# jonasrothfuss/meta_learning_pacoh

Measured on AMD Instinct MI355X. Metric: task-GP LML+grad evals/sec (n_ctx=64, d=4, 20 particles), higher is better.
Workload: dtype f32; 1 GPU; PACOH-SVGD step as meta_fit runs it (hipGraph replay), cfg#3: 1024 tasks per GPU x 20 particles, n_ctx=64, d=4, NN(32,32) mean + NN(32,32) kernel (D=2534), task sharding + 1 all-reduce/step; parallelism=task-shard x1, finite=True, tasks_total=1024, particles=20, n_ctx=64, d=4

## Files before the change

meta_learning_pacoh_amd/csrc/gp_fwd_reg.hip:

```cpp
#include "gp_reg_body.h"
#include "mlp_act.h"
#include "step_tail.h"
#include "switches.h"

namespace pacoh {

struct FwdGpArgs {
    const float* x;
    const float* theta; long theta_stride;
    long off_mean, off_kern;
    float* stash_mean; float* stash_kern;
    int d_in, h0, h1;
    int nblk;
    unsigned n_prob;
    SvgdDistTail<float> sv;
};

namespace gpreg {

struct FwdCtx : KernelCtx {
    static constexpr bool LDS_INPUTS = true;
    __device__ __forceinline__ int lane() const { int l = threadIdx.x; asm volatile("" : "+v"(l)); return l; }
};

__device__ __forceinline__ void dist_tail_wave(const SvgdDistTail<float>& t, int lin, int nlin) {
    const int lane = threadIdx.x;
    if (lin == 0 && lane == 0 && t.counter) *t.counter += 1;
    for (int pair = lin; pair < t.P * t.P; pair += nlin) {
        const int i = pair / t.P, j = pair - i * t.P;
        if (j > i) continue;
        const float* xi = t.X + (long)i * t.D;
        if (t.snap && i == j) {
            for (int d = lane; d < t.D; d += 64) t.snap[(long)i * t.D + d] = xi[d];
            if (lane == 0) t.d2[i * t.P + i] = 0.0f;
            continue;
        }
        const float* xj = t.X + (long)j * t.D;
        float acc[4] = {0.0f, 0.0f, 0.0f, 0.0f};
        for (int d0 = lane; d0 < t.D; d0 += 256) {
#pragma unroll
            for (int w = 0; w < 4; ++w) {
                const int d = d0 + 64 * w;
                if (d < t.D) { const float df = xi[d] - xj[d]; acc[w] = fmaf(df, df, acc[w]); }
            }
        }
#pragma unroll
        for (int w = 0; w < 4; ++w) acc[w] = subwave_sum<float>(acc[w], 64);
        if (lane == 0) { const float tot = (acc[0] + acc[1]) + (acc[2] + acc[3]); t.d2[i * t.P + j] = tot; t.d2[j * t.P + i] = tot; }
    }
}

template <int NH, bool W32, bool MEAN>
__device__ __forceinline__ void fwd_net(const float* __restrict__ th, const FwdGpArgs& fa, int d_out, const float (&bx)[4], float* stash,
                                        long blk0, int lane, float* zf, float* rv) {
    const int r = lane & 15, g = lane >> 4;
    const int h0 = W32 ? 32 : fa.h0, d_in = fa.d_in;
    float aw1[2];
    f32x4 b1[2];
#pragma unroll
    for (int fb = 0; fb < 2; ++fb) {
        const int o = fb * 16 + r;
        aw1[fb] = ((W32 || o < h0) && g < d_in) ? TSC * th[h0 + o * d_in + g] : 0.0f;
#pragma unroll
        for (int s = 0; s < 4; ++s) { const int q = fb * 16 + 4 * g + s; b1[fb][s] = (W32 || q < h0) ? TSC * th[q] : 0.0f; }
    }
    int src = h0 * (d_in + 1), prev = h0;
    f32x4 aw2[2][2], b2[2];
    if constexpr (NH == 2) {
        const int hl = W32 ? 32 : fa.h1;
#pragma unroll
        for (int ob = 0; ob < 2; ++ob) {
            const int o = ob * 16 + r;
#pragma unroll
            for (int kb = 0; kb < 2; ++kb)
#pragma unroll
                for (int j = 0; j < 4; ++j) {
                    const int k = kb * 16 + 4 * g + j;
                    aw2[ob][kb][j] = (W32 || (o < hl && k < prev)) ? TSC * th[src + hl + o * prev + k] : 0.0f;
                }
#pragma unroll
            for (int s = 0; s < 4; ++s) { const int q = ob * 16 + 4 * g + s; b2[ob][s] = (W32 || q < hl) ? TSC * th[src + q] : 0.0f; }
        }
        src += hl * (prev + 1);
        prev = hl;
    }
    constexpr int NO = MEAN ? 1 : 2;
    float w3[NO][2][4], b3[NO];
#pragma unroll
    for (int o = 0; o < NO; ++o) {
        b3[o] = o < d_out ? th[src + o] : 0.0f;
#pragma unroll
        for (int fb = 0; fb < 2; ++fb)
#pragma unroll
            for (int s = 0; s < 4; ++s) {
                const int k = fb * 16 + 4 * g + s;
                w3[o][fb][s] = (o < d_out && (W32 || k < prev)) ? th[src + d_out + o * prev + k] : 0.0f;
            }
    }
#pragma unroll
    for (int pb = 0; pb < 4; ++pb) {
        asm volatile("" ::: "memory"); __builtin_amdgcn_sched_barrier(0);
        f32x4 HA[2], HB[2];
#pragma unroll
        for (int fb = 0; fb < 2; ++fb) {
            f32x4 acc = mfma_(aw1[fb], bx[pb], b1[fb]);
#pragma unroll
            for (int s = 0; s < 4; ++s) acc[s] = tanh_pre(acc[s]);
            HA[fb] = acc;
        }
        if constexpr (NH == 2) {
#pragma unroll
            for (int ob = 0; ob < 2; ++ob) {
                f32x4 acc = b2[ob];
#pragma unroll
                for (int kb = 0; kb < 2; ++kb) {
                    acc = mfma_(aw2[ob][kb][0], HA[kb][0], acc); acc = mfma_(aw2[ob][kb][1], HA[kb][1], acc);
                    acc = mfma_(aw2[ob][kb][2], HA[kb][2], acc); acc = mfma_(aw2[ob][kb][3], HA[kb][3], acc);
                }
#pragma unroll
                for (int s = 0; s < 4; ++s) acc[s] = tanh_pre(acc[s]);
                HB[ob] = acc;
            }
            if (stash) {
#pragma unroll
                for (int fb = 0; fb < 2; ++fb)
                    __builtin_nontemporal_store(HB[fb], reinterpret_cast<f32x4*>(stash + ((((blk0 + pb) * 2 + fb) << 8) + (lane << 2))));
            }
        }
        const f32x4 (&HL)[2] = NH == 2 ? HB : HA;
        float v[NO];
#pragma unroll
        for (int o = 0; o < NO; ++o) v[o] = 0.0f;
#pragma unroll
        for (int fb = 0; fb < 2; ++fb)
#pragma unroll
            for (int s = 0; s < 4; ++s)
#pragma unroll
                for (int o = 0; o < NO; ++o) v[o] = fmaf(w3[o][fb][s], HL[fb][s], v[o]);
#pragma unroll
        for (int o = 0; o < NO; ++o) { v[o] += __shfl_xor(v[o], 16, 64); v[o] += __shfl_xor(v[o], 32, 64); }
        if (g == 0) {
            if constexpr (MEAN) rv[pb * 16 + r] = v[0] + b3[0];
            else {
                zf[(pb * 16 + r) * 2] = v[0] + b3[0];
                if (d_out > 1) zf[(pb * 16 + r) * 2 + 1] = v[1] + b3[1];
            }
        }
    }
}

}

template <int NH, bool W32>
__global__ void __launch_bounds__(64, 4) gp_fwd_reg_kernel(GpMfmaArgs a, FwdGpArgs fa) {
    if (blockIdx.x >= fa.n_prob) {
        gpreg::dist_tail_wave(fa.sv, (int)(blockIdx.x - fa.n_prob), (int)(gridDim.x - fa.n_prob));
        return;
    }
    if (const int32_t* n_act = gpreg::KernelCtx{}.late(a.n_act, (unsigned)__builtin_offsetof(GpMfmaArgs, n_act))) {
        if (blockIdx.x >= (unsigned)*n_act * (unsigned)a.P) return;
    }
    constexpr int NB = 4, FP = 2, NP = 16 * NB, NU = NB * (NB + 1) / 2;
    __shared__ __attribute__((aligned(16))) float zf[NP * FP];
    __shared__ __attribute__((aligned(16))) float rv[NP];
    __shared__ __attribute__((aligned(16))) float av[NP];
    __shared__ __attribute__((aligned(16))) float fsc[gpreg::GPR_SCR];
    float* tsc = fsc;
    __shared__ __attribute__((aligned(16))) float dzc[NP * FP];
    __shared__ __attribute__((aligned(16))) float Wl[(NU - NB) * 256];
    {
        const int lane = threadIdx.x, r = lane & 15, g = lane >> 4;
        const unsigned t = blockIdx.x / (unsigned)a.P, p = blockIdx.x - t * (unsigned)a.P;
        const float* xt = fa.x + (long)t * NP * fa.d_in;
        float bx[4];
#pragma unroll
        for (int pb = 0; pb < 4; ++pb) bx[pb] = g < fa.d_in ? xt[(pb * 16 + r) * fa.d_in + g] : 0.0f;
        const float* th = fa.theta + (long)p * fa.theta_stride;
        const long blk0 = (long)p * fa.nblk + 4 * t;
        gpreg::fwd_net<NH, W32, true>(th + fa.off_mean, fa, 1, bx, fa.stash_mean, blk0, lane, zf, rv);
        asm volatile("" ::: "memory"); __builtin_amdgcn_sched_barrier(0);
        gpreg::fwd_net<NH, W32, false>(th + fa.off_kern, fa, a.f, bx, fa.stash_kern, blk0, lane, zf, rv);
        asm volatile("" ::: "memory"); __builtin_amdgcn_wave_barrier();
    }
    gpreg::gp_reg_body<NB, FP, true, false>(a, gpreg::FwdCtx{}, zf, rv, av, fsc, tsc, dzc, Wl);
}

static bool fwd_gp_applicable(int B, int P, int n, int x_div, int d_in, const int32_t* hidden, int n_hidden, int f_arg, int has_os,
                              int mean_mode, int dtype) {
    if (dtype != PACOH_F32 || kernel_of(f_arg) != PACOH_KERNEL_RBF || has_os || mean_mode != PACOH_MEAN_VECTOR) return false;
    const int f = features_of(f_arg);
    if (f < 1 || f > 2 || n != 64 || P <= 0 || B <= 0 || B % P != 0 || x_div != P || d_in < 1 || d_in > 4) return false;
    if (n_hidden < 1 || n_hidden > 2 || !hidden || g_sw.mlp_path != 0) return false;
    for (int l = 0; l < n_hidden; ++l) if (hidden[l] < 1 || hidden[l] > 32) return false;
    return (long)B * n <= 0x3fffffffL;
}

}

using namespace pacoh;

extern "C" int pacoh_fwd_gp_applicable(int B, int P, int n, int x_div, int d_in, const int32_t* hidden, int n_hidden, int f,
                                       int has_outputscale, int mean_mode, int dtype) {
    return fwd_gp_applicable(B, P, n, x_div, d_in, hidden, n_hidden, f, has_outputscale, mean_mode, dtype) ? 1 : 0;
}

extern "C" int pacoh_fwd_gp_lml_fwdbwd(const pacoh_active_tasks* act, const void* x, int x_div, const void* theta, long theta_stride, int P,
                                       int d_in, const int32_t* hidden, int n_hidden, long off_mean, long off_kernel, void* stash,
                                       const void* svgd_X, void* svgd_workspace, int svgd_P, int svgd_D, int64_t* counter,
                                       const void* y, int y_div, const void* lengthscale, const void* outputscale, const void* noise,
                                       const int32_t* n_valid, const void* g_lml, void* lml, void* d_z, void* d_mean,
                                       void* d_lengthscale, void* d_outputscale, void* d_noise, int32_t* info,
                                       int B, int n, int f, int dtype, void* stream) {
    if (check_dtype(dtype)) return PACOH_EDTYPE;
    if (!x || !theta || !y || !lengthscale || !noise || !lml || !d_lengthscale || !d_noise || y_div <= 0 || off_mean < 0 || off_kernel < 0)
        return PACOH_EINVAL;
    if (act && (!act->n_act || !act->task_w)) return PACOH_EINVAL;
    if (svgd_X && (!svgd_workspace || svgd_P <= 0 || svgd_D <= 0)) return PACOH_EINVAL;
    if (svgd_X && svgd_P > PACOH_SVGD_MAX_PARTICLES) return PACOH_ELIMIT;
    if (!fwd_gp_applicable(B, P, n, x_div, d_in, hidden, n_hidden, f, outputscale != nullptr || d_outputscale != nullptr,
                           PACOH_MEAN_VECTOR, dtype))
        return PACOH_ELIMIT;
    GpMfmaArgs a = {nullptr, 1, nullptr, PACOH_MEAN_VECTOR, (const float*)y, y_div, (const float*)lengthscale, nullptr, (const float*)noise,
                    n_valid, (const float*)g_lml, (float*)lml, info, (float*)d_z, (float*)d_mean, (float*)d_lengthscale, nullptr,
                    (float*)d_noise, B, P, n, features_of(f)};
    if (act) { a.n_act = act->n_act; a.task_w = (const float*)act->task_w; }
    FwdGpArgs fa = {};
    fa.x = (const float*)x; fa.theta = (const float*)theta; fa.theta_stride = theta_stride;
    fa.off_mean = off_mean; fa.off_kern = off_kernel;
    fa.d_in = d_in; fa.h0 = hidden[0]; fa.h1 = n_hidden > 1 ? hidden[1] : 0;
    fa.nblk = 4 * (B / P);
    if (stash && n_hidden > 1) {
        fa.stash_mean = (float*)stash;
        fa.stash_kern = (float*)stash + (size_t)P * fa.nblk * 2 * 256;
    }
    fa.n_prob = (unsigned)B;
    unsigned tail_wgs = 0;
    if (svgd_X) {
        float* d2 = (float*)svgd_workspace;
        fa.sv = SvgdDistTail<float>{(const float*)svgd_X, d2, d2 + svgd_P * svgd_P, svgd_P, svgd_D, (long*)counter};
        tail_wgs = (unsigned)(svgd_P * svgd_P);
    }
    const bool w32 = hidden[0] == 32 && (n_hidden == 1 || hidden[1] == 32);
    const dim3 grid((unsigned)B + tail_wgs);
    hipStream_t s = (hipStream_t)stream;
    if (n_hidden == 2) {
        if (w32) hipLaunchKernelGGL((gp_fwd_reg_kernel<2, true>), grid, dim3(64), 0, s, a, fa);
        else hipLaunchKernelGGL((gp_fwd_reg_kernel<2, false>), grid, dim3(64), 0, s, a, fa);
    } else {
        if (w32) hipLaunchKernelGGL((gp_fwd_reg_kernel<1, true>), grid, dim3(64), 0, s, a, fa);
        else hipLaunchKernelGGL((gp_fwd_reg_kernel<1, false>), grid, dim3(64), 0, s, a, fa);
    }
    return launch_status();
}
```

meta_learning_pacoh_amd/csrc/mlp_fused.hip:

```cpp
#include "common.h"
#include "hyper_tail.h"
#include "step_tail.h"
#include "mlp_fused_split.h"
#include "mlp_act.h"
#include <stdlib.h>

namespace pacoh {

using f32x4 = __attribute__((ext_vector_type(4))) float;

constexpr int FMAXNH = 4;
constexpr int LWH = 36;
constexpr int HBLK = 32 * LWH + 32;
constexpr int F_OFF_W1 = 0;
constexpr int F_OFF_B1 = 128;
constexpr int F_OFF_H = 160;
__host__ __device__ constexpr int f_off_out(int nh) { return F_OFF_H + (nh - 1) * HBLK; }
__host__ __device__ constexpr int f_welems(int nh) { return f_off_out(nh) + 68; }
__host__ __device__ constexpr int f_dnet_max(int nh) { return 32 * 5 + (nh - 1) * 32 * 33 + 2 * 33; }
__host__ __device__ constexpr bool bwd_wg_slab(int nh) { return nh <= 2; }
constexpr int TSTRIDE = 4;
constexpr int TSTAGE = 6;
constexpr int TLD = 17;
__host__ __device__ constexpr int tskew(int k) { return 12 * (k & 1) + 32 * (k >> 1); }
constexpr int TRS = 320;

struct FusedNet {
    long theta_off;
    float* out;
    const float* g_out;
    float* slab;
    float* stash;
    int d_out, D_net;
};

struct FusedArgs {
    const float* x; int x_div;
    const float* theta; long theta_stride;
    FusedNet net[2];
    int P, n, R;
    int d_in, nh;
    int h[FMAXNH];
    int tiles_per_wg;
    int n_stash;
    int nblk;
    int tail_z;
    SvgdDistTail<float> sv;
    const float* bw_d2; float* bw_out; int bw_P;
    long* adv_counter;
    const int32_t* n_act;
    int tiles;
};

__device__ __forceinline__ void fused_live_rows(const FusedArgs& a, int tp, int& R, int& tpw) {
    R = a.R; tpw = a.tiles_per_wg;
    if (!a.n_act) return;
    const int live = *a.n_act * a.n;
    if (live < R) R = live;
    tpw = fused_split_tiles((R + tp - 1) / tp, a.tiles, (int)gridDim.x, tpw);
}

__device__ __forceinline__ long stash_off(const FusedArgs& a, int p, int blk, int slot, int fb, int lane) {
    return (((((long)p * a.nblk + blk) * a.n_stash + slot) * 2 + fb) << 8) + (lane << 2);
}

__device__ __forceinline__ f32x4 fmfma(float a, float b, f32x4 c) {
    return __builtin_amdgcn_mfma_f32_16x16x4f32(a, b, c, 0, 0, 0);
}


template <int NH>
__device__ void fused_load_weights(float* wl, const float* __restrict__ th, const FusedArgs& a, int d_out) {
    for (int q = threadIdx.x; q < f_welems(NH); q += blockDim.x) wl[q] = 0.0f;
    __syncthreads();
    int src = 0;
    const int h0 = a.h[0], d_in = a.d_in;
    for (int q = threadIdx.x; q < h0; q += blockDim.x) wl[F_OFF_B1 + q] = TSC * th[q];
    for (int q = threadIdx.x; q < h0 * d_in; q += blockDim.x) { const int o = q / d_in, k = q - o * d_in; wl[F_OFF_W1 + o * 4 + k] = TSC * th[h0 + q]; }
    src += h0 * (d_in + 1);
    int prev = h0;
#pragma unroll
    for (int l = 1; l < NH; ++l) {
        const int hl = a.h[l];
        float* dst = wl + F_OFF_H + (l - 1) * HBLK;
        for (int q = threadIdx.x; q < hl; q += blockDim.x) dst[32 * LWH + q] = TSC * th[src + q];
        for (int q = threadIdx.x; q < hl * prev; q += blockDim.x) { const int o = q / prev, k = q - o * prev; dst[o * LWH + k] = TSC * th[src + hl + q]; }
        src += hl * (prev + 1);
        prev = hl;
    }
    float* dst = wl + f_off_out(NH);
    for (int q = threadIdx.x; q < d_out; q += blockDim.x) dst[64 + q] = th[src + q];
    for (int q = threadIdx.x; q < d_out * prev; q += blockDim.x) { const int o = q / prev, k = q - o * prev; dst[o * 32 + k] = th[src + d_out + q]; }
    __syncthreads();
}

template <int PB, bool BWD>
__device__ __forceinline__ long stage_tile(const FusedArgs& a, const FusedNet& nt, int p, int row0, float* st, int lane, int R) {
    long orow = -1;
    if (lane < 16 * PB) {
        const int row = row0 + lane;
        const bool valid = row < R;
        const int rr = valid ? row : R - 1;
        const int t = (int)((unsigned)rr / (unsigned)a.n), i = rr - t * a.n;
        const int bi = t * a.P + p;
        const int xb = a.x_div == 1 ? bi : (int)((unsigned)bi / (unsigned)a.x_div);
        const float* xq = a.x + ((long)xb * a.n + i) * (long)a.d_in;
        float4 xv;
        xv.x = xq[0];
        xv.y = a.d_in > 1 ? xq[1] : 0.0f;
        xv.z = a.d_in > 2 ? xq[2] : 0.0f;
        xv.w = a.d_in > 3 ? xq[3] : 0.0f;
        *reinterpret_cast<float4*>(st + lane * TSTRIDE) = xv;
        const long o = (long)bi * a.n + i;
        if (BWD) {
            const float* gq = nt.g_out + o * nt.d_out;
            st[16 * PB * TSTRIDE + lane] = valid ? gq[0] : 0.0f;
            st[16 * PB * (TSTRIDE + 1) + lane] = (valid && nt.d_out > 1) ? gq[1] : 0.0f;
        }
        orow = valid ? o : -1;
    }
    asm volatile("" ::: "memory");
    return orow;
}

template <int PB>
__device__ __forceinline__ void f_layer1(const float* wl, const float* st, int r, int g, f32x4 (&H)[2][PB]) {
    float bx[PB];
#pragma unroll
    for (int pb = 0; pb < PB; ++pb) bx[pb] = st[(pb * 16 + r) * TSTRIDE + g];
#pragma unroll
    for (int fb = 0; fb < 2; ++fb) {
        f32x4 bias;
#pragma unroll
        for (int s = 0; s < 4; ++s) bias[s] = wl[F_OFF_B1 + fb * 16 + 4 * g + s];
        const float aw = wl[F_OFF_W1 + (fb * 16 + r) * 4 + g];
#pragma unroll
        for (int pb = 0; pb < PB; ++pb) {
            f32x4 acc = fmfma(aw, bx[pb], bias);
#pragma unroll
            for (int s = 0; s < 4; ++s) acc[s] = tanh_pre(acc[s]);
            H[fb][pb] = acc;
        }
    }
}

template <int PB>
__device__ __forceinline__ void f_hidden(const float* W, int r, int g, const f32x4 (&IN)[2][PB], f32x4 (&OUT)[2][PB]) {
#pragma unroll
    for (int ob = 0; ob < 2; ++ob) {
        f32x4 bias;
#pragma unroll
        for (int s = 0; s < 4; ++s) bias[s] = W[32 * LWH + ob * 16 + 4 * g + s];
#pragma unroll
        for (int pb = 0; pb < PB; ++pb) OUT[ob][pb] = bias;
#pragma unroll
        for (int kb = 0; kb < 2; ++kb) {
            const float4 aw = *reinterpret_cast<const float4*>(W + (ob * 16 + r) * LWH + kb * 16 + 4 * g);
#pragma unroll
            for (int pb = 0; pb < PB; ++pb) {
                f32x4 acc = OUT[ob][pb];
                acc = fmfma(aw.x, IN[kb][pb][0], acc); acc = fmfma(aw.y, IN[kb][pb][1], acc);
                acc = fmfma(aw.z, IN[kb][pb][2], acc); acc = fmfma(aw.w, IN[kb][pb][3], acc);
                OUT[ob][pb] = acc;
            }
        }
#pragma unroll
        for (int pb = 0; pb < PB; ++pb)
#pragma unroll
            for (int s = 0; s < 4; ++s) OUT[ob][pb][s] = tanh_pre(OUT[ob][pb][s]);
    }
}

template <int PB>
__device__ __forceinline__ void f_delta(const float* W, int r, int g, const f32x4 (&DOUT)[2][PB], f32x4 (&HIN)[2][PB]) {
#pragma unroll
    for (int fb = 0; fb < 2; ++fb) {
        f32x4 acc[PB];
#pragma unroll
        for (int pb = 0; pb < PB; ++pb) acc[pb] = f32x4{0.f, 0.f, 0.f, 0.f};
#pragma unroll
        for (int ob = 0; ob < 2; ++ob) {
            const float* wp = W + (ob * 16 + 4 * g) * LWH + fb * 16 + r;
            const float a0 = wp[0], a1 = wp[LWH], a2 = wp[2 * LWH], a3 = wp[3 * LWH];
#pragma unroll
            for (int pb = 0; pb < PB; ++pb) {
                acc[pb] = fmfma(a0, DOUT[ob][pb][0], acc[pb]); acc[pb] = fmfma(a1, DOUT[ob][pb][1], acc[pb]);
                acc[pb] = fmfma(a2, DOUT[ob][pb][2], acc[pb]); acc[pb] = fmfma(a3, DOUT[ob][pb][3], acc[pb]);
            }
        }
#pragma unroll
        for (int pb = 0; pb < PB; ++pb)
#pragma unroll
            for (int s = 0; s < 4; ++s) { const float h = HIN[fb][pb][s]; HIN[fb][pb][s] = acc[pb][s] * (1.0f - h * h); }
    }
}

__device__ __forceinline__ f32x4 f_turn(float* scr, const f32x4& v, int wr, int rd) {
    f32x4 o;
#pragma unroll
    for (int s = 0; s < 4; ++s) scr[wr + s * TLD] = v[s];
    asm volatile("" ::: "memory");
#pragma unroll
    for (int q = 0; q < 4; ++q) o[q] = scr[rd + q];
    asm volatile("" ::: "memory");
    return o;
}

__device__ __forceinline__ void f_wgrad(f32x4& acc, const f32x4& Ap, const f32x4& Bp) {
    acc = fmfma(Ap[0], Bp[0], acc); acc = fmfma(Ap[1], Bp[1], acc);
    acc = fmfma(Ap[2], Bp[2], acc); acc = fmfma(Ap[3], Bp[3], acc);
}

__device__ __forceinline__ void stash_st(const f32x4& v, f32x4* q) {
    __builtin_nontemporal_store(v, q);
}
__device__ __forceinline__ f32x4 stash_ld(const f32x4* q) {
    return *q;
}

template <int PB>
__device__ __forceinline__ void stash_put(const FusedArgs& a, const FusedNet& nt, int p, int blk0, int slot, int lane,
                                          const f32x4 (&H)[2][PB]) {
#pragma unroll
    for (int pb = 0; pb < PB; ++pb)
#pragma unroll
        for (int fb = 0; fb < 2; ++fb)
            stash_st(H[fb][pb], reinterpret_cast<f32x4*>(nt.stash + stash_off(a, p, blk0 + pb, slot, fb, lane)));
}

template <int PB>
__device__ __forceinline__ void stash_get(const FusedArgs& a, const FusedNet& nt, int p, int blk0, int slot, int lane,
                                          f32x4 (&H)[2][PB], int R) {
#pragma unroll
    for (int pb = 0; pb < PB; ++pb) {
        const bool in = (blk0 + pb) * 16 < R;
#pragma unroll
        for (int fb = 0; fb < 2; ++fb)
            H[fb][pb] = in ? stash_ld(reinterpret_cast<const f32x4*>(nt.stash + stash_off(a, p, blk0 + pb, slot, fb, lane)))
                           : f32x4{0.f, 0.f, 0.f, 0.f};
    }
}

template <int NH, int PB, int MINW>
__global__ void __launch_bounds__(256, MINW) mlp_fused_fwd_kernel(FusedArgs a) {
    __shared__ __attribute__((aligned(16))) float wl[f_welems(NH)];
    __shared__ __attribute__((aligned(16))) float stage[4][16 * PB * TSTAGE];
    if (a.tail_z > 0 && (int)blockIdx.z == a.tail_z) {
        svgd_dist_tail<float>(a.sv, (int)(blockIdx.y * gridDim.x + blockIdx.x), (int)(gridDim.x * gridDim.y));
        return;
    }
    int R, tpw;
    fused_live_rows(a, 16 * PB, R, tpw);
    const FusedNet& nt = a.net[blockIdx.z];
    const int p = blockIdx.y;
    fused_load_weights<NH>(wl, a.theta + (long)p * a.theta_stride + nt.theta_off, a, nt.d_out);
    const int lane = threadIdx.x & 63, wave = __builtin_amdgcn_readfirstlane(threadIdx.x >> 6);
    const int r = lane & 15, g = lane >> 4;
    float* st = stage[wave];
    const float* wo = wl + f_off_out(NH);
    float w3r[2][2][4];
#pragma unroll
    for (int o = 0; o < 2; ++o)
#pragma unroll
        for (int fb = 0; fb < 2; ++fb)
#pragma unroll
            for (int s = 0; s < 4; ++s) w3r[o][fb][s] = wo[o * 32 + fb * 16 + 4 * g + s];
    const float b30 = wo[64], b31 = wo[65];
    constexpr int TP = 16 * PB;
    for (int tl = wave; tl < tpw; tl += 4) {
        const int row0 = (blockIdx.x * tpw + tl) * TP;
        if (row0 >= R) break;
        const long orow_l = stage_tile<PB, false>(a, nt, p, row0, st, lane, R);
        f32x4 HA[2][PB], HB[2][PB];
        const int blk0 = row0 >> 4;
        const int ns = nt.stash ? a.n_stash : 0;
        f_layer1<PB>(wl, st, r, g, HA);
        if (ns >= NH) stash_put<PB>(a, nt, p, blk0, 0, lane, HA);
#pragma unroll
        for (int l = 1; l < NH; ++l) {
            if (l & 1) f_hidden<PB>(wl + F_OFF_H + (l - 1) * HBLK, r, g, HA, HB);
            else f_hidden<PB>(wl + F_OFF_H + (l - 1) * HBLK, r, g, HB, HA);
            if (l >= NH - ns) stash_put<PB>(a, nt, p, blk0, l - (NH - ns), lane, (l & 1) ? HB : HA);
        }
        const f32x4 (&HL)[2][PB] = ((NH - 1) & 1) ? HB : HA;
#pragma unroll
        for (int pb = 0; pb < PB; ++pb) {
            float v0 = 0.f, v1 = 0.f;
#pragma unroll
            for (int fb = 0; fb < 2; ++fb)
#pragma unroll
                for (int s = 0; s < 4; ++s) { v0 = fmaf(w3r[0][fb][s], HL[fb][pb][s], v0); v1 = fmaf(w3r[1][fb][s], HL[fb][pb][s], v1); }
            v0 += __shfl_xor(v0, 16, 64); v0 += __shfl_xor(v0, 32, 64);
            v1 += __shfl_xor(v1, 16, 64); v1 += __shfl_xor(v1, 32, 64);
            const long orow = __shfl(orow_l, pb * 16 + r, 64);
            if (g == 0 && orow >= 0) {
                nt.out[orow * nt.d_out] = v0 + b30;
                if (nt.d_out > 1) nt.out[orow * nt.d_out + 1] = v1 + b31;
            }
        }
    }
}

template <int NH, int PB, int MINW>
__global__ void __launch_bounds__(256, MINW) mlp_fused_bwd_kernel(FusedArgs a) {
    constexpr int L_WL = (f_welems(NH) + 3) & ~3, L_ST = 4 * 16 * PB * TSTAGE, L_TS = 4 * 2 * TRS;
    constexpr int L_RED = bwd_wg_slab(NH) ? 4 * f_dnet_max(NH) : 0;
    constexpr int L_ALL = (L_WL + L_ST + L_TS) > L_RED ? (L_WL + L_ST + L_TS) : L_RED;
    __shared__ __attribute__((aligned(16))) float lds[L_ALL];
    if (a.tail_z > 0 && (int)blockIdx.z == a.tail_z) {
        if (blockIdx.x == 0 && blockIdx.y == 0) {
            if (a.bw_out) svgd_bandwidth_block<float>(a.bw_d2, a.bw_P, a.bw_out);
            if (a.adv_counter && threadIdx.x == 0) *a.adv_counter += 1;
        }
        return;
    }
    int R, tpw;
    fused_live_rows(a, 16 * PB, R, tpw);
    float* wl = lds;
    const FusedNet& nt = a.net[blockIdx.z];
    const int p = blockIdx.y;
    fused_load_weights<NH>(wl, a.theta + (long)p * a.theta_stride + nt.theta_off, a, nt.d_out);
    const int lane = threadIdx.x & 63, wave = __builtin_amdgcn_readfirstlane(threadIdx.x >> 6);
    const int r = lane & 15, g = lane >> 4;
    float* st = lds + L_WL + wave * (16 * PB * TSTAGE);
    float* sc0 = lds + L_WL + L_ST + wave * (2 * TRS);
    float* sc1 = sc0 + TRS;
    const int twr = 4 * TLD * g + tskew(g) + r, trd = TLD * r + tskew(r >> 2) + 4 * g;
    const float* wo = wl + f_off_out(NH);

    f32x4 aW[NH > 1 ? NH - 1 : 1][2][2] = {};
    float aBh[NH > 1 ? NH - 1 : 1][2] = {};
    float aW1[2][4] = {}, aB1[2] = {};
    f32x4 aWoT[2][2] = {};
    float aBoT[2] = {};

    constexpr int TP = 16 * PB;
    for (int tl = wave; tl < tpw; tl += 4) {
        const int row0 = (blockIdx.x * tpw + tl) * TP;
        if (row0 >= R) break;
        stage_tile<PB, true>(a, nt, p, row0, st, lane, R);
        f32x4 H[NH][2][PB];
        const int blk0 = row0 >> 4;
        const int ns = nt.stash ? a.n_stash : 0;
#pragma unroll
        for (int l = NH - 1; l >= 0; --l)
            if (l >= NH - ns) stash_get<PB>(a, nt, p, blk0, l - (NH - ns), lane, H[l], R);
        if (ns < NH) f_layer1<PB>(wl, st, r, g, H[0]);
#pragma unroll
        for (int l = 1; l < NH; ++l)
            if (l < NH - ns) f_hidden<PB>(wl + F_OFF_H + (l - 1) * HBLK, r, g, H[l - 1], H[l]);
        {
            f32x4 w3[2][2];
#pragma unroll
            for (int o = 0; o < 2; ++o)
#pragma unroll
                for (int fb = 0; fb < 2; ++fb) w3[o][fb] = *reinterpret_cast<const f32x4*>(wo + o * 32 + fb * 16 + 4 * g);
#pragma unroll
            for (int pb = 0; pb < PB; ++pb) {
                float2 gr;
                gr.x = st[16 * PB * TSTRIDE + pb * 16 + r];
                gr.y = st[16 * PB * (TSTRIDE + 1) + pb * 16 + r];
                aBoT[0] += gr.x; aBoT[1] += gr.y;
#pragma unroll
                for (int fb = 0; fb < 2; ++fb)
#pragma unroll
                    for (int s = 0; s < 4; ++s) {
                        const float h = H[NH - 1][fb][pb][s];
                        aWoT[0][fb][s] = fmaf(gr.x, h, aWoT[0][fb][s]);
                        aWoT[1][fb][s] = fmaf(gr.y, h, aWoT[1][fb][s]);
                        const float d = fmaf(w3[1][fb][s], gr.y, w3[0][fb][s] * gr.x);
                        H[NH - 1][fb][pb][s] = d * (1.0f - h * h);
                    }
            }
        }
#pragma unroll
        for (int l = NH - 1; l >= 1; --l) {
#pragma unroll
            for (int pb = 0; pb < PB; ++pb) {
                f32x4 Dp[2], Hp[2];
                Dp[0] = f_turn(sc0, H[l][0][pb], twr, trd);     Hp[0] = f_turn(sc1, H[l - 1][0][pb], twr, trd);
                Dp[1] = f_turn(sc0, H[l][1][pb], twr, trd);     Hp[1] = f_turn(sc1, H[l - 1][1][pb], twr, trd);
#pragma unroll
                for (int ob = 0; ob < 2; ++ob) {
                    aBh[l - 1][ob] += (Dp[ob][0] + Dp[ob][1]) + (Dp[ob][2] + Dp[ob][3]);
#pragma unroll
                    for (int kb = 0; kb < 2; ++kb) f_wgrad(aW[l - 1][ob][kb], Dp[ob], Hp[kb]);
                }
            }
            f_delta<PB>(wl + F_OFF_H + (l - 1) * HBLK, r, g, H[l], H[l - 1]);
        }
#pragma unroll
        for (int pb = 0; pb < PB; ++pb) {
            const f32x4 Dp0 = f_turn(sc0, H[0][0][pb], twr, trd);
            const f32x4 Dp1 = f_turn(sc1, H[0][1][pb], twr, trd);
#pragma unroll
            for (int q = 0; q < 4; ++q) {
                const float4 xp = *reinterpret_cast<const float4*>(st + (pb * 16 + 4 * g + q) * TSTRIDE);
                aW1[0][0] = fmaf(Dp0[q], xp.x, aW1[0][0]); aW1[0][1] = fmaf(Dp0[q], xp.y, aW1[0][1]);
                aW1[0][2] = fmaf(Dp0[q], xp.z, aW1[0][2]); aW1[0][3] = fmaf(Dp0[q], xp.w, aW1[0][3]);
                aW1[1][0] = fmaf(Dp1[q], xp.x, aW1[1][0]); aW1[1][1] = fmaf(Dp1[q], xp.y, aW1[1][1]);
                aW1[1][2] = fmaf(Dp1[q], xp.z, aW1[1][2]); aW1[1][3] = fmaf(Dp1[q], xp.w, aW1[1][3]);
                aB1[0] += Dp0[q]; aB1[1] += Dp1[q];
            }
        }
    }
    auto rg = [](float v) { v += __shfl_xor(v, 16, 64); v += __shfl_xor(v, 32, 64); return v; };
    if (bwd_wg_slab(NH)) __syncthreads();
    float* dst = bwd_wg_slab(NH) ? lds + wave * nt.D_net : nt.slab + ((long)(blockIdx.x * 4 + wave) * a.P + p) * nt.D_net;
    const int d_in = a.d_in, h0 = a.h[0];
    float unscale[NH];
    unscale[NH - 1] = 1.0f;
#pragma unroll
    for (int j = NH - 2; j >= 0; --j) unscale[j] = unscale[j + 1] * INV_TSC;
#pragma unroll
    for (int fb = 0; fb < 2; ++fb) {
        const int o = fb * 16 + r;
        const float b = rg(aB1[fb]) * unscale[0];
        if (g == 0 && o < h0) dst[o] = b;
#pragma unroll
        for (int k = 0; k < 4; ++k) { const float v = rg(aW1[fb][k]) * unscale[0]; if (g == 0 && o < h0 && k < d_in) dst[h0 + o * d_in + k] = v; }
    }
    int off = h0 * (d_in + 1), prev = h0;
#pragma unroll
    for (int l = 1; l < NH; ++l) {
        const int hl = a.h[l];
#pragma unroll
        for (int ob = 0; ob < 2; ++ob) {
            const float b = rg(aBh[l - 1][ob]) * unscale[l];
            if (g == 0 && ob * 16 + r < hl) dst[off + ob * 16 + r] = b;
#pragma unroll
            for (int kb = 0; kb < 2; ++kb)
#pragma unroll
                for (int s = 0; s < 4; ++s) {
                    const int o = ob * 16 + 4 * g + s, k = kb * 16 + r;
                    if (o < hl && k < prev) dst[off + hl + o * prev + k] = aW[l - 1][ob][kb][s] * unscale[l];
                }
        }
        off += hl * (prev + 1);
        prev = hl;
    }
    auto rs = [](float v) {
        v += __shfl_xor(v, 1, 64); v += __shfl_xor(v, 2, 64); v += __shfl_xor(v, 4, 64); v += __shfl_xor(v, 8, 64);
        return v;
    };
#pragma unroll
    for (int o = 0; o < 2; ++o) {
        const float b = rs(aBoT[o]);
        if (lane == 0 && o < nt.d_out) dst[off + o] = b;
#pragma unroll
        for (int fb = 0; fb < 2; ++fb)
#pragma unroll
            for (int s = 0; s < 4; ++s) {
                const float v = rs(aWoT[o][fb][s]);
                const int k = fb * 16 + 4 * g + s;
                if (r == 0 && o < nt.d_out && k < prev) dst[off + nt.d_out + o * prev + k] = v;
            }
    }
    if (bwd_wg_slab(NH)) {
        __syncthreads();
        float* out = nt.slab + ((long)blockIdx.x * a.P + p) * nt.D_net;
        for (int e = threadIdx.x; e < nt.D_net; e += 256)
            out[e] = (lds[e] + lds[nt.D_net + e]) + (lds[2 * nt.D_net + e] + lds[3 * nt.D_net + e]);
    }
}

struct SlabReduce { const float* in; float* out; int Wd; int col0; };
template <int LSH>
__global__ void __launch_bounds__(256) fused_reduce_slab_kernel(SlabReduce s0, SlabReduce s1, long out_stride, int accumulate, int C, int P,
                                                                int nets, HyperBwdArgs<float> tail, int tail_blocks, float* img_th, const int* img_map) {
    constexpr int LANES = 1 << LSH;
    if ((int)blockIdx.y == nets) {
        __shared__ float red[4];
        if ((int)blockIdx.x < tail_blocks) hyper_tail_block<float>(tail, blockIdx.x, red);
// ... 235 lines not shown
```

Baseline: 64.32 million evals/s.

## Share per-particle NN weight images in LDS across four task waves per workgroup

The forward GP kernel now runs four waves per workgroup, each handling a different task for the same particle. The mean and kernel network weights are loaded cooperatively once into LDS (aliased over two waves' scratch) instead of every single-wave block gathering them from global memory into registers. The per-point MLP evaluation then uses the shared LDS-based layer helpers, processing four point blocks at a time, and the SVGD distance tail is remapped to one pair per wave. This adds a workgroup barrier and larger blocks, with possible occupancy and tail-imbalance effects when the task count is not a multiple of four.

```diff
diff --git a/meta_learning_pacoh_amd/csrc/gp_fwd_reg.hip b/meta_learning_pacoh_amd/csrc/gp_fwd_reg.hip
--- a/meta_learning_pacoh_amd/csrc/gp_fwd_reg.hip
+++ b/meta_learning_pacoh_amd/csrc/gp_fwd_reg.hip
@@ -1,5 +1,5 @@
 #include "gp_reg_body.h"
-#include "mlp_act.h"
+#include "mlp_fwd_lds.h"
 #include "step_tail.h"
 #include "switches.h"
 
@@ -10,21 +10,28 @@
     const float* theta; long theta_stride;
     long off_mean, off_kern;
     float* stash_mean; float* stash_kern;
-    int d_in, h0, h1;
+    int d_in, h[2];
     int nblk;
-    unsigned n_prob;
+    int T;
+    unsigned n_wg;
     SvgdDistTail<float> sv;
 };
 
 namespace gpreg {
 
+constexpr int FWD_WAVES = 4;
+constexpr int FWD_PB = 4;
+static_assert(FWD_PB == 1 || FWD_PB == 2 || FWD_PB == 4, "a 64-point problem is four 16-point blocks");
+
 struct FwdCtx : KernelCtx {
     static constexpr bool LDS_INPUTS = true;
-    __device__ __forceinline__ int lane() const { int l = threadIdx.x; asm volatile("" : "+v"(l)); return l; }
+    unsigned b;
+    __device__ __forceinline__ int lane() const { return threadIdx.x & 63; }
+    __device__ __forceinline__ unsigned block() const { return b; }
 };
 
 __device__ __forceinline__ void dist_tail_wave(const SvgdDistTail<float>& t, int lin, int nlin) {
-    const int lane = threadIdx.x;
+    const int lane = threadIdx.x & 63;
     if (lin == 0 && lane == 0 && t.counter) *t.counter += 1;
     for (int pair = lin; pair < t.P * t.P; pair += nlin) {
         const int i = pair / t.P, j = pair - i * t.P;
@@ -50,139 +57,183 @@
     }
 }
 
-template <int NH, bool W32, bool MEAN>
-__device__ __forceinline__ void fwd_net(const float* __restrict__ th, const FwdGpArgs& fa, int d_out, const float (&bx)[4], float* stash,
-                                        long blk0, int lane, float* zf, float* rv) {
+template <int NH, bool W32, int NT>
+struct WeightImage {
+    static constexpr int NSMALL = 128 + 32 + 32 + 64 + 4, TURNS = (NSMALL + NT - 1) / NT, WTURNS = NH == 2 ? 256 / NT : 1;
+    f32x4 w[WTURNS];
+    float v[TURNS];
+    bool w_ok[WTURNS][4], v_ok[TURNS];
+    __device__ __forceinline__ void fetch(const float* __restrict__ th, int d_in, int h0_, int h1_, int d_out, int tid) {
+        const int h0 = W32 ? 32 : h0_, h1 = W32 ? 32 : h1_;
+        const int src1 = h0 * (d_in + 1);
+        const int src_o = NH == 2 ? src1 + h1 * (h0 + 1) : src1, prev = NH == 2 ? h1 : h0;
+        if constexpr (NH == 2) {
+#pragma unroll
+            for (int it = 0; it < WTURNS; ++it) {
+                const int c = tid + NT * it, o = c >> 3, k0 = (c & 7) * 4;
+#pragma unroll
+                for (int j = 0; j < 4; ++j) {
+                    const bool ok = (o < h1) & (k0 + j < h0);
+                    w[it][j] = th[ok ? src1 + h1 + o * h0 + k0 + j : 0];
+                    w_ok[it][j] = ok;
+                }
+            }
+        }
+#pragma unroll
+        for (int it = 0; it < TURNS; ++it) {
+            const int q = tid + NT * it;
+            const int o1 = q >> 2, k1 = q & 3, e = q - 192, o3 = e >> 5, k3 = e & 31;
+            const bool ok_w1 = (o1 < h0) & (k1 < d_in), ok_b1 = q - 128 < h0, ok_b2 = q - 160 < h1, ok_wo = (o3 < d_out) & (k3 < prev), ok_bo = q - 256 < d_out;
+            const int i_w1 = h0 + o1 * d_in + k1, i_b1 = q - 128, i_b2 = src1 + q - 160, i_wo = src_o + d_out + o3 * prev + k3, i_bo = src_o + q - 256;
+            bool ok = ok_bo; int idx = i_bo;
+            if (q < 256) { ok = ok_wo; idx = i_wo; }
+            if (q < 192) { ok = ok_b2; idx = i_b2; }
+            if (q < 160) { ok = ok_b1; idx = i_b1; }
+            if (q < 128) { ok = ok_w1; idx = i_w1; }
+            v[it] = th[ok ? idx : 0];
+            v_ok[it] = ok;
+        }
+    }
+    __device__ __forceinline__ void put(float* wl, int tid) const {
+        if constexpr (NH == 2) {
+#pragma unroll
+            for (int it = 0; it < WTURNS; ++it) {
+                const int c = tid + NT * it;
+                f32x4 x = w[it];
+                asm volatile("" : "+v"(x));
+#pragma unroll
+                for (int j = 0; j < 4; ++j) x[j] = w_ok[it][j] ? TSC * x[j] : 0.0f;
+                *reinterpret_cast<f32x4*>(wl + F_OFF_H + (c >> 3) * LWH + (c & 7) * 4) = x;
+            }
+        }
+#pragma unroll
+        for (int it = 0; it < TURNS; ++it) {
+            const int q = tid + NT * it;
+            const int dst = q < 160 ? q : q < 192 ? F_OFF_H + 32 * LWH + q - 160 : f_off_out(NH) + q - 192;
+            const bool mine = (q < NSMALL) & (NH == 2 || q < 160 || q >= 192);
+            float x = v[it];
+            asm volatile("" : "+v"(x));
+            x = q < 192 ? TSC * x : x;
+            wl[mine ? dst : f_off_out(NH) + 67] = (mine & v_ok[it]) ? x : 0.0f;
+        }
+    }
+};
+static_assert(F_OFF_W1 == 0 && F_OFF_B1 == 128, "WeightImage::put");
+
+template <int NH, bool MEAN>
+__device__ __forceinline__ void fwd_net(const float* wl, int d_out, const float (&bx)[4], float* stash, long blk0, int lane, float* zf,
+                                        float* rv) {
     const int r = lane & 15, g = lane >> 4;
-    const int h0 = W32 ? 32 : fa.h0, d_in = fa.d_in;
-    float aw1[2];
-    f32x4 b1[2];
-#pragma unroll
-    for (int fb = 0; fb < 2; ++fb) {
-        const int o = fb * 16 + r;
-        aw1[fb] = ((W32 || o < h0) && g < d_in) ? TSC * th[h0 + o * d_in + g] : 0.0f;
-#pragma unroll
-        for (int s = 0; s < 4; ++s) { const int q = fb * 16 + 4 * g + s; b1[fb][s] = (W32 || q < h0) ? TSC * th[q] : 0.0f; }
-    }
-    int src = h0 * (d_in + 1), prev = h0;
-    f32x4 aw2[2][2], b2[2];
-    if constexpr (NH == 2) {
-        const int hl = W32 ? 32 : fa.h1;
-#pragma unroll
-        for (int ob = 0; ob < 2; ++ob) {
-            const int o = ob * 16 + r;
-#pragma unroll
-            for (int kb = 0; kb < 2; ++kb)
-#pragma unroll
-                for (int j = 0; j < 4; ++j) {
-                    const int k = kb * 16 + 4 * g + j;
-                    aw2[ob][kb][j] = (W32 || (o < hl && k < prev)) ? TSC * th[src + hl + o * prev + k] : 0.0f;
+    constexpr int NO = MEAN ? 1 : 2;
+    const float* wo = wl + f_off_out(NH);
+    f32x4 w3[NO][2];
+    float b3[NO];
+#pragma unroll
+    for (int o = 0; o < NO; ++o) {
+        b3[o] = wo[64 + o];
+#pragma unroll
+        for (int fb = 0; fb < 2; ++fb) w3[o][fb] = *reinterpret_cast<const f32x4*>(wo + o * 32 + fb * 16 + 4 * g);
+    }
+#pragma unroll
+    for (int p0 = 0; p0 < 4; p0 += FWD_PB) {
+        asm volatile("" ::: "memory"); __builtin_amdgcn_sched_barrier(0);
+        float bxg[FWD_PB];
+#pragma unroll
+        for (int pb = 0; pb < FWD_PB; ++pb) bxg[pb] = bx[p0 + pb];
+        f32x4 HA[2][FWD_PB], HB[2][FWD_PB];
+        f_layer1_bx<FWD_PB>(wl, bxg, r, g, HA);
+        if constexpr (NH == 2) {
+            f_hidden<FWD_PB>(wl + F_OFF_H, r, g, HA, HB);
+            if (stash) {
+#pragma unroll
+                for (int pb = 0; pb < FWD_PB; ++pb)
+#pragma unroll
+                    for (int fb = 0; fb < 2; ++fb)
+                        __builtin_nontemporal_store(HB[fb][pb], reinterpret_cast<f32x4*>(stash + ((((blk0 + p0 + pb) * 2 + fb) << 8) + (lane << 2))));
+            }
+        }
+        const f32x4 (&HL)[2][FWD_PB] = NH == 2 ? HB : HA;
+#pragma unroll
+        for (int pb = 0; pb < FWD_PB; ++pb) {
+            float v[NO];
+#pragma unroll
+            for (int o = 0; o < NO; ++o) v[o] = 0.0f;
+#pragma unroll
+            for (int fb = 0; fb < 2; ++fb)
+#pragma unroll
+                for (int s = 0; s < 4; ++s)
+#pragma unroll
+                    for (int o = 0; o < NO; ++o) v[o] = fmaf(w3[o][fb][s], HL[fb][pb][s], v[o]);
+#pragma unroll
+            for (int o = 0; o < NO; ++o) { v[o] += __shfl_xor(v[o], 16, 64); v[o] += __shfl_xor(v[o], 32, 64); }
+            if (g == 0) {
+                const int pt = (p0 + pb) * 16 + r;
+                if constexpr (MEAN) rv[pt] = v[0] + b3[0];
+                else {
+                    zf[pt * 2] = v[0] + b3[0];
+                    if (d_out > 1) zf[pt * 2 + 1] = v[1] + b3[1];
                 }
-#pragma unroll
-            for (int s = 0; s < 4; ++s) { const int q = ob * 16 + 4 * g + s; b2[ob][s] = (W32 || q < hl) ? TSC * th[src + q] : 0.0f; }
-        }
-        src += hl * (prev + 1);
-        prev = hl;
-    }
-    constexpr int NO = MEAN ? 1 : 2;
-    float w3[NO][2][4], b3[NO];
-#pragma unroll
-    for (int o = 0; o < NO; ++o) {
-        b3[o] = o < d_out ? th[src + o] : 0.0f;
-#pragma unroll
-        for (int fb = 0; fb < 2; ++fb)
-#pragma unroll
-            for (int s = 0; s < 4; ++s) {
-                const int k = fb * 16 + 4 * g + s;
-                w3[o][fb][s] = (o < d_out && (W32 || k < prev)) ? th[src + d_out + o * prev + k] : 0.0f;
-            }
-    }
-#pragma unroll
-    for (int pb = 0; pb < 4; ++pb) {
+            }
+        }
+    }
+}
+
+}
+
+template <int NH, bool W32>
+__global__ void __launch_bounds__(64 * gpreg::FWD_WAVES, 4) gp_fwd_reg_kernel(GpMfmaArgs a, FwdGpArgs fa) {
+    constexpr int NW = gpreg::FWD_WAVES;
+    if (blockIdx.x >= fa.n_wg) {
+        gpreg::dist_tail_wave(fa.sv, (int)(blockIdx.x - fa.n_wg) * NW + (int)(threadIdx.x >> 6), (int)(gridDim.x - fa.n_wg) * NW);
+        return;
+    }
+    int T = fa.T;
+    if (const int32_t* n_act = gpreg::KernelCtx{}.late(a.n_act, (unsigned)__builtin_offsetof(GpMfmaArgs, n_act))) {
+        const int na = *n_act;
+        if (na < T) T = na;
+    }
+    const unsigned tg = __builtin_amdgcn_readfirstlane(blockIdx.x / (unsigned)a.P), p = blockIdx.x - tg * (unsigned)a.P;
+    if ((int)(NW * tg) >= T) return;
+    constexpr int NB = 4, FP = 2, NP = 16 * NB, NU = NB * (NB + 1) / 2, WLN = (NU - NB) * 256;
+    constexpr int O_ZF = 0, O_RV = O_ZF + NP * FP, O_AV = O_RV + NP, O_FSC = O_AV + NP, O_DZC = O_FSC + gpreg::GPR_SCR, O_WL = O_DZC + NP * FP;
+    constexpr int WAVE_LDS = O_WL + WLN;
+    __shared__ __attribute__((aligned(16))) float lds[NW][WAVE_LDS];
+    static_assert(f_welems(NH) <= WLN && NW >= 2, "a network's weight image aliases one wave's Wl");
+    static_assert(WAVE_LDS * sizeof(float) == 8960 && O_WL % 4 == 0 && O_FSC % 4 == 0, "8 960 bytes of LDS per problem: 16 problems per CU");
+    const int wave = __builtin_amdgcn_readfirstlane(threadIdx.x >> 6);
+    float* wl_mean = lds[0] + O_WL;
+    float* wl_kern = lds[1] + O_WL;
+    float* my = lds[wave];
+    const unsigned t = NW * tg + (unsigned)wave;
+    const bool live = (int)t < T;
+    const int lane = threadIdx.x & 63;
+    float bx[4];
+    {
+        const int r = lane & 15, g = lane >> 4;
+        const float* xt = fa.x + (long)(live ? t : 0u) * NP * fa.d_in;
+#pragma unroll
+        for (int pb = 0; pb < 4; ++pb) bx[pb] = xt[g < fa.d_in ? (pb * 16 + r) * fa.d_in + g : 0];
+        const float* th = fa.theta + (long)p * fa.theta_stride;
+        gpreg::WeightImage<NH, W32, 64 * NW> im_mean, im_kern;
+        im_mean.fetch(th + fa.off_mean, fa.d_in, fa.h[0], fa.h[1], 1, threadIdx.x);
+        im_kern.fetch(th + fa.off_kern, fa.d_in, fa.h[0], fa.h[1], a.f, threadIdx.x);
+        im_mean.put(wl_mean, threadIdx.x);
+        im_kern.put(wl_kern, threadIdx.x);
+        __syncthreads();
+#pragma unroll
+        for (int pb = 0; pb < 4; ++pb) { asm volatile("" : "+v"(bx[pb])); bx[pb] = g < fa.d_in ? bx[pb] : 0.0f; }
+    }
+    if (live) {
+        const long blk0 = (long)p * fa.nblk + 4 * t;
+        gpreg::fwd_net<NH, true>(wl_mean, 1, bx, fa.stash_mean, blk0, lane, my + O_ZF, my + O_RV);
         asm volatile("" ::: "memory"); __builtin_amdgcn_sched_barrier(0);
-        f32x4 HA[2], HB[2];
-#pragma unroll
-        for (int fb = 0; fb < 2; ++fb) {
-            f32x4 acc = mfma_(aw1[fb], bx[pb], b1[fb]);
-#pragma unroll
-            for (int s = 0; s < 4; ++s) acc[s] = tanh_pre(acc[s]);
-            HA[fb] = acc;
-        }
-        if constexpr (NH == 2) {
-#pragma unroll
-            for (int ob = 0; ob < 2; ++ob) {
-                f32x4 acc = b2[ob];
-#pragma unroll
-                for (int kb = 0; kb < 2; ++kb) {
-                    acc = mfma_(aw2[ob][kb][0], HA[kb][0], acc); acc = mfma_(aw2[ob][kb][1], HA[kb][1], acc);
-                    acc = mfma_(aw2[ob][kb][2], HA[kb][2], acc); acc = mfma_(aw2[ob][kb][3], HA[kb][3], acc);
-                }
-#pragma unroll
-                for (int s = 0; s < 4; ++s) acc[s] = tanh_pre(acc[s]);
-                HB[ob] = acc;
-            }
-            if (stash) {
-#pragma unroll
-                for (int fb = 0; fb < 2; ++fb)
-                    __builtin_nontemporal_store(HB[fb], reinterpret_cast<f32x4*>(stash + ((((blk0 + pb) * 2 + fb) << 8) + (lane << 2))));
-            }
-        }
-        const f32x4 (&HL)[2] = NH == 2 ? HB : HA;
-        float v[NO];
-#pragma unroll
-        for (int o = 0; o < NO; ++o) v[o] = 0.0f;
-#pragma unroll
-        for (int fb = 0; fb < 2; ++fb)
-#pragma unroll
-            for (int s = 0; s < 4; ++s)
-#pragma unroll
-                for (int o = 0; o < NO; ++o) v[o] = fmaf(w3[o][fb][s], HL[fb][s], v[o]);
-#pragma unroll
-        for (int o = 0; o < NO; ++o) { v[o] += __shfl_xor(v[o], 16, 64); v[o] += __shfl_xor(v[o], 32, 64); }
-        if (g == 0) {
-            if constexpr (MEAN) rv[pb * 16 + r] = v[0] + b3[0];
-            else {
-                zf[(pb * 16 + r) * 2] = v[0] + b3[0];
-                if (d_out > 1) zf[(pb * 16 + r) * 2 + 1] = v[1] + b3[1];
-            }
-        }
-    }
-}
-
-}
-
-template <int NH, bool W32>
-__global__ void __launch_bounds__(64, 4) gp_fwd_reg_kernel(GpMfmaArgs a, FwdGpArgs fa) {
-    if (blockIdx.x >= fa.n_prob) {
-        gpreg::dist_tail_wave(fa.sv, (int)(blockIdx.x - fa.n_prob), (int)(gridDim.x - fa.n_prob));
-        return;
-    }
-    if (const int32_t* n_act = gpreg::KernelCtx{}.late(a.n_act, (unsigned)__builtin_offsetof(GpMfmaArgs, n_act))) {
-        if (blockIdx.x >= (unsigned)*n_act * (unsigned)a.P) return;
-    }
-    constexpr int NB = 4, FP = 2, NP = 16 * NB, NU = NB * (NB + 1) / 2;
-    __shared__ __attribute__((aligned(16))) float zf[NP * FP];
-    __shared__ __attribute__((aligned(16))) float rv[NP];
-    __shared__ __attribute__((aligned(16))) float av[NP];
-    __shared__ __attribute__((aligned(16))) float fsc[gpreg::GPR_SCR];
-    float* tsc = fsc;
-    __shared__ __attribute__((aligned(16))) float dzc[NP * FP];
-    __shared__ __attribute__((aligned(16))) float Wl[(NU - NB) * 256];
-    {
-        const int lane = threadIdx.x, r = lane & 15, g = lane >> 4;
-        const unsigned t = blockIdx.x / (unsigned)a.P, p = blockIdx.x - t * (unsigned)a.P;
-        const float* xt = fa.x + (long)t * NP * fa.d_in;
-        float bx[4];
-#pragma unroll
-        for (int pb = 0; pb < 4; ++pb) bx[pb] = g < fa.d_in ? xt[(pb * 16 + r) * fa.d_in + g] : 0.0f;
-        const float* th = fa.theta + (long)p * fa.theta_stride;
-        const long blk0 = (long)p * fa.nblk + 4 * t;
-        gpreg::fwd_net<NH, W32, true>(th + fa.off_mean, fa, 1, bx, fa.stash_mean, blk0, lane, zf, rv);
-        asm volatile("" ::: "memory"); __builtin_amdgcn_sched_barrier(0);
-        gpreg::fwd_net<NH, W32, false>(th + fa.off_kern, fa, a.f, bx, fa.stash_kern, blk0, lane, zf, rv);
-        asm volatile("" ::: "memory"); __builtin_amdgcn_wave_barrier();
-    }
-    gpreg::gp_reg_body<NB, FP, true, false>(a, gpreg::FwdCtx{}, zf, rv, av, fsc, tsc, dzc, Wl);
+        gpreg::fwd_net<NH, false>(wl_kern, a.f, bx, fa.stash_kern, blk0, lane, my + O_ZF, my + O_RV);
+    }
+    __syncthreads();
+    if (!live) return;
+    gpreg::FwdCtx cx;
+    cx.b = t * (unsigned)a.P + p;
+    gpreg::gp_reg_body<NB, FP, true, false>(a, cx, my + O_ZF, my + O_RV, my + O_AV, my + O_FSC, my + O_FSC, my + O_DZC, my + O_WL);
 }
 
 static bool fwd_gp_applicable(int B, int P, int n, int x_div, int d_in, const int32_t* hidden, int n_hidden, int f_arg, int has_os,
@@ -227,28 +278,29 @@
     FwdGpArgs fa = {};
     fa.x = (const float*)x; fa.theta = (const float*)theta; fa.theta_stride = theta_stride;
     fa.off_mean = off_mean; fa.off_kern = off_kernel;
-    fa.d_in = d_in; fa.h0 = hidden[0]; fa.h1 = n_hidden > 1 ? hidden[1] : 0;
+    fa.d_in = d_in; fa.h[0] = hidden[0]; fa.h[1] = n_hidden > 1 ? hidden[1] : 0;
     fa.nblk = 4 * (B / P);
     if (stash && n_hidden > 1) {
         fa.stash_mean = (float*)stash;
         fa.stash_kern = (float*)stash + (size_t)P * fa.nblk * 2 * 256;
     }
-    fa.n_prob = (unsigned)B;
+    fa.T = B / P;
+    fa.n_wg = (unsigned)((fa.T + gpreg::FWD_WAVES - 1) / gpreg::FWD_WAVES) * (unsigned)P;
     unsigned tail_wgs = 0;
     if (svgd_X) {
         float* d2 = (float*)svgd_workspace;
         fa.sv = SvgdDistTail<float>{(const float*)svgd_X, d2, d2 + svgd_P * svgd_P, svgd_P, svgd_D, (long*)counter};
-        tail_wgs = (unsigned)(svgd_P * svgd_P);
-    }
+        tail_wgs = (unsigned)((svgd_P * svgd_P + gpreg::FWD_WAVES - 1) / gpreg::FWD_WAVES);
+    }
+    const dim3 grid(fa.n_wg + tail_wgs), block(64 * gpreg::FWD_WAVES);
+    hipStream_t s = (hipStream_t)stream;
     const bool w32 = hidden[0] == 32 && (n_hidden == 1 || hidden[1] == 32);
-    const dim3 grid((unsigned)B + tail_wgs);
-    hipStream_t s = (hipStream_t)stream;
     if (n_hidden == 2) {
-        if (w32) hipLaunchKernelGGL((gp_fwd_reg_kernel<2, true>), grid, dim3(64), 0, s, a, fa);
-        else hipLaunchKernelGGL((gp_fwd_reg_kernel<2, false>), grid, dim3(64), 0, s, a, fa);
+        if (w32) hipLaunchKernelGGL((gp_fwd_reg_kernel<2, true>), grid, block, 0, s, a, fa);
+        else hipLaunchKernelGGL((gp_fwd_reg_kernel<2, false>), grid, block, 0, s, a, fa);
     } else {
-        if (w32) hipLaunchKernelGGL((gp_fwd_reg_kernel<1, true>), grid, dim3(64), 0, s, a, fa);
-        else hipLaunchKernelGGL((gp_fwd_reg_kernel<1, false>), grid, dim3(64), 0, s, a, fa);
+        if (w32) hipLaunchKernelGGL((gp_fwd_reg_kernel<1, true>), grid, block, 0, s, a, fa);
+        else hipLaunchKernelGGL((gp_fwd_reg_kernel<1, false>), grid, block, 0, s, a, fa);
     }
     return launch_status();
 }
diff --git a/meta_learning_pacoh_amd/csrc/mlp_fused.hip b/meta_learning_pacoh_amd/csrc/mlp_fused.hip
--- a/meta_learning_pacoh_amd/csrc/mlp_fused.hip
+++ b/meta_learning_pacoh_amd/csrc/mlp_fused.hip
@@ -2,21 +2,12 @@
 #include "hyper_tail.h"
 #include "step_tail.h"
 #include "mlp_fused_split.h"
-#include "mlp_act.h"
+#include "mlp_fwd_lds.h"
 #include <stdlib.h>
 
 namespace pacoh {
 
-using f32x4 = __attribute__((ext_vector_type(4))) float;
-
 constexpr int FMAXNH = 4;
-constexpr int LWH = 36;
-constexpr int HBLK = 32 * LWH + 32;
-constexpr int F_OFF_W1 = 0;
-constexpr int F_OFF_B1 = 128;
-constexpr int F_OFF_H = 160;
-__host__ __device__ constexpr int f_off_out(int nh) { return F_OFF_H + (nh - 1) * HBLK; }
-__host__ __device__ constexpr int f_welems(int nh) { return f_off_out(nh) + 68; }
 __host__ __device__ constexpr int f_dnet_max(int nh) { return 32 * 5 + (nh - 1) * 32 * 33 + 2 * 33; }
 __host__ __device__ constexpr bool bwd_wg_slab(int nh) { return nh <= 2; }
 constexpr int TSTRIDE = 4;
@@ -62,10 +53,6 @@
 
 __device__ __forceinline__ long stash_off(const FusedArgs& a, int p, int blk, int slot, int fb, int lane) {
     return (((((long)p * a.nblk + blk) * a.n_stash + slot) * 2 + fb) << 8) + (lane << 2);
-}
-
-__device__ __forceinline__ f32x4 fmfma(float a, float b, f32x4 c) {
-    return __builtin_amdgcn_mfma_f32_16x16x4f32(a, b, c, 0, 0, 0);
 }
 
 
@@ -128,47 +115,7 @@
     float bx[PB];
 #pragma unroll
     for (int pb = 0; pb < PB; ++pb) bx[pb] = st[(pb * 16 + r) * TSTRIDE + g];
-#pragma unroll
-    for (int fb = 0; fb < 2; ++fb) {
-        f32x4 bias;
-#pragma unroll
-        for (int s = 0; s < 4; ++s) bias[s] = wl[F_OFF_B1 + fb * 16 + 4 * g + s];
-        const float aw = wl[F_OFF_W1 + (fb * 16 + r) * 4 + g];
-#pragma unroll
-        for (int pb = 0; pb < PB; ++pb) {
-            f32x4 acc = fmfma(aw, bx[pb], bias);
-#pragma unroll
-            for (int s = 0; s < 4; ++s) acc[s] = tanh_pre(acc[s]);
-            H[fb][pb] = acc;
-        }
-    }
-}
-
-template <int PB>
-__device__ __forceinline__ void f_hidden(const float* W, int r, int g, const f32x4 (&IN)[2][PB], f32x4 (&OUT)[2][PB]) {
-#pragma unroll
-    for (int ob = 0; ob < 2; ++ob) {
-        f32x4 bias;
-#pragma unroll
-        for (int s = 0; s < 4; ++s) bias[s] = W[32 * LWH + ob * 16 + 4 * g + s];
-#pragma unroll
-        for (int pb = 0; pb < PB; ++pb) OUT[ob][pb] = bias;
-#pragma unroll
-        for (int kb = 0; kb < 2; ++kb) {
-            const float4 aw = *reinterpret_cast<const float4*>(W + (ob * 16 + r) * LWH + kb * 16 + 4 * g);
-#pragma unroll
-            for (int pb = 0; pb < PB; ++pb) {
-                f32x4 acc = OUT[ob][pb];
-                acc = fmfma(aw.x, IN[kb][pb][0], acc); acc = fmfma(aw.y, IN[kb][pb][1], acc);
-                acc = fmfma(aw.z, IN[kb][pb][2], acc); acc = fmfma(aw.w, IN[kb][pb][3], acc);
-                OUT[ob][pb] = acc;
-            }
-        }
-#pragma unroll
-        for (int pb = 0; pb < PB; ++pb)
-#pragma unroll
-            for (int s = 0; s < 4; ++s) OUT[ob][pb][s] = tanh_pre(OUT[ob][pb][s]);
-    }
+    f_layer1_bx<PB>(wl, bx, r, g, H);
 }
 
 template <int PB>
diff --git a/meta_learning_pacoh_amd/csrc/mlp_fwd_lds.h b/meta_learning_pacoh_amd/csrc/mlp_fwd_lds.h
--- /dev/null
+++ b/meta_learning_pacoh_amd/csrc/mlp_fwd_lds.h
@@ -0,0 +1,65 @@
+#pragma once
+#include "mlp_act.h"
+
+namespace pacoh {
+
+using f32x4 = __attribute__((ext_vector_type(4))) float;
+
+constexpr int LWH = 36;
+constexpr int HBLK = 32 * LWH + 32;
+constexpr int F_OFF_W1 = 0;
+constexpr int F_OFF_B1 = 128;
+constexpr int F_OFF_H = 160;
+__host__ __device__ constexpr int f_off_out(int nh) { return F_OFF_H + (nh - 1) * HBLK; }
+__host__ __device__ constexpr int f_welems(int nh) { return f_off_out(nh) + 68; }
+
+__device__ __forceinline__ f32x4 fmfma(float a, float b, f32x4 c) {
+    return __builtin_amdgcn_mfma_f32_16x16x4f32(a, b, c, 0, 0, 0);
+}
+
+template <int PB>
+__device__ __forceinline__ void f_layer1_bx(const float* wl, const float (&bx)[PB], int r, int g, f32x4 (&H)[2][PB]) {
+#pragma unroll
+    for (int fb = 0; fb < 2; ++fb) {
+        f32x4 bias;
+#pragma unroll
+        for (int s = 0; s < 4; ++s) bias[s] = wl[F_OFF_B1 + fb * 16 + 4 * g + s];
+        const float aw = wl[F_OFF_W1 + (fb * 16 + r) * 4 + g];
+#pragma unroll
+        for (int pb = 0; pb < PB; ++pb) {
+            f32x4 acc = fmfma(aw, bx[pb], bias);
+#pragma unroll
+            for (int s = 0; s < 4; ++s) acc[s] = tanh_pre(acc[s]);
+            H[fb][pb] = acc;
+        }
+    }
+}
+
+template <int PB>
+__device__ __forceinline__ void f_hidden(const float* W, int r, int g, const f32x4 (&IN)[2][PB], f32x4 (&OUT)[2][PB]) {
+#pragma unroll
+    for (int ob = 0; ob < 2; ++ob) {
+        f32x4 bias;
+#pragma unroll
+        for (int s = 0; s < 4; ++s) bias[s] = W[32 * LWH + ob * 16 + 4 * g + s];
+#pragma unroll
+        for (int pb = 0; pb < PB; ++pb) OUT[ob][pb] = bias;
+#pragma unroll
+        for (int kb = 0; kb < 2; ++kb) {
+            const float4 aw = *reinterpret_cast<const float4*>(W + (ob * 16 + r) * LWH + kb * 16 + 4 * g);
+#pragma unroll
+            for (int pb = 0; pb < PB; ++pb) {
+                f32x4 acc = OUT[ob][pb];
+                acc = fmfma(aw.x, IN[kb][pb][0], acc); acc = fmfma(aw.y, IN[kb][pb][1], acc);
+                acc = fmfma(aw.z, IN[kb][pb][2], acc); acc = fmfma(aw.w, IN[kb][pb][3], acc);
+                OUT[ob][pb] = acc;
+            }
+        }
+#pragma unroll
+        for (int pb = 0; pb < PB; ++pb)
+#pragma unroll
+            for (int s = 0; s < 4; ++s) OUT[ob][pb][s] = tanh_pre(OUT[ob][pb][s]);
+    }
+}
+
+}
```

Result: slower. 59.67 million evals/s (-7.2%).
